# uncbiag/OAI_analysis_2

Measured on AMD Instinct MI355X. Metric: knee MRI volumes/sec (segment+register), 384x384x160 fp32, higher is better.
Workload: dtype fp16x3 (every fp32 value held as 2 fp16 terms = 22 mantissa bits, 3 MFMA passes per product, fp32 accumulate; fp32 in and out of every entry point; full-size parity vs the reference in `parity`)

## Files before the change

oai_analysis_2_amd/csrc/icon.hip:

```cpp
#include <cmath>
#include <cstring>
#include <vector>

#include "common.h"

namespace {

constexpr int kDown[6] = {2, 16, 32, 64, 256, 512};
constexpr int kUpOut[5] = {16, 32, 64, 128, 256};
constexpr int kUpIn[5] = {48, 96, 192, 512, 512};
constexpr float kLeaky = 0.01f;
constexpr float kBnEps = 1e-5f;
constexpr long long kSplitKBelow = 16384;
constexpr long long kMfmaUpFrom = 2048;
#ifndef OAI_LAST_XT
#define OAI_LAST_XT 2
#endif
constexpr long long kFewBlocks = 1024;

__device__ __forceinline__ float leaky(float v) { return v > 0.0f ? v : v * kLeaky; }

struct __attribute__((packed, aligned(4))) pair_f32s { float a, b; };
__device__ __forceinline__ void pair_store(float* p, float a, float b) { *reinterpret_cast<pair_f32s*>(p) = pair_f32s{a, b}; }

// ... 66 lines not shown

__device__ __forceinline__ void up_src(int dst, int in_size, int& i0, int& i1, float& l0, float& l1) {
    float src = 0.5f * ((float)dst + 0.5f) - 0.5f;
    src = src < 0.0f ? 0.0f : src;
    i0 = (int)src;
    i1 = i0 + (i0 < in_size - 1 ? 1 : 0);
    l1 = src - (float)i0;
    l0 = 1.0f - l1;
}

template <int COUT_T, int KS>
__global__ void __launch_bounds__(256)
icon_up_kernel(const float* __restrict__ x, int Cin, int D, int H, int W,
               const float* __restrict__ wk , const float* __restrict__ bias,
               const float* __restrict__ bn_scale, const float* __restrict__ bn_shift,
               float* __restrict__ out, int Cout, int Dc, int Hc, int Wc) {
    constexpr int VT = 256 / KS;
    __shared__ float red[KS > 1 ? (KS - 1) * VT * COUT_T : 1];
    const int cg = blockIdx.y;
    const int ks = KS == 1 ? 0 : threadIdx.x / VT;
    const int par = blockIdx.z, pz = par >> 2, py = (par >> 1) & 1, px = par & 1;
    const int nz = (Dc - pz + 1) / 2, ny = (Hc - py + 1) / 2, nx = (Wc - px + 1) / 2;
    const long long nv = (long long)nz * ny * nx;
    const long long v = (long long)blockIdx.x * VT + threadIdx.x % VT;
    const bool live = v < nv;
    const long long vv = live ? v : 0;
    const int tx = (int)(vv % nx), ty = (int)((vv / nx) % ny), tz = (int)(vv / ((long long)nx * ny));
    const int oz = 2 * tz + pz, oy = 2 * ty + py, ox = 2 * tx + px;
    const long long plane = (long long)D * H * W;
    const long long oplane = (long long)Dc * Hc * Wc;
    const int qz = (pz + 1) & 1, qy = (py + 1) & 1, qx = (px + 1) & 1;
    float acc[COUT_T];
#pragma unroll
    for (int j = 0; j < COUT_T; ++j) acc[j] = 0.0f;
    if (KS == 1 && !live) return;
    if (KS == 1 || live)
        for (int ci = ks; ci < Cin; ci += KS) {
            const float* xp = x + ci * plane;
            const float* wp = wk + ((long long)ci * 64) * Cout + cg * COUT_T;
#pragma unroll 8
            for (int t = 0; t < 8; ++t) {
                const int kz = qz + 2 * (t >> 2), ky = qy + 2 * ((t >> 1) & 1), kx = qx + 2 * (t & 1);
                const int iz = (oz + 1 - kz) >> 1, iy = (oy + 1 - ky) >> 1, ix = (ox + 1 - kx) >> 1;
                float in = 0.0f;
                if ((unsigned)iz < (unsigned)D && (unsigned)iy < (unsigned)H && (unsigned)ix < (unsigned)W)
                    in = leaky(xp[((long long)iz * H + iy) * W + ix]);
                const float* w = wp + ((kz * 4 + ky) * 4 + kx) * Cout;
#pragma unroll
                for (int j = 0; j < COUT_T; ++j) acc[j] = fmaf(in, w[j], acc[j]);
            }
        }
    if (KS > 1) {
        if (ks > 0) {
#pragma unroll
            for (int j = 0; j < COUT_T; ++j) red[((ks - 1) * COUT_T + j) * VT + threadIdx.x % VT] = acc[j];
        }
        __syncthreads();
        if (ks > 0) return;
#pragma unroll
        for (int k = 1; k < KS; ++k)
#pragma unroll
            for (int j = 0; j < COUT_T; ++j) acc[j] += red[((k - 1) * COUT_T + j) * VT + threadIdx.x];
    }
    if (!live) return;
    int z0, z1, y0, y1, x0, x1;
    float a0, a1, b0, b1, c0, c1;
    up_src(oz, D, z0, z1, a0, a1);
    up_src(oy, H, y0, y1, b0, b1);
    up_src(ox, W, x0, x1, c0, c1);
#pragma unroll
    for (int j = 0; j < COUT_T; ++j) {
        const int co = cg * COUT_T + j;
        const float* p = x + co * plane;
        auto at = [&](int zz, int yy, int xx) { return p[((long long)zz * H + yy) * W + xx]; };
        const float res = a0 * (b0 * (c0 * at(z0, y0, x0) + c1 * at(z0, y0, x1)) + b1 * (c0 * at(z0, y1, x0) + c1 * at(z0, y1, x1))) +
                          a1 * (b0 * (c0 * at(z1, y0, x0) + c1 * at(z1, y0, x1)) + b1 * (c0 * at(z1, y1, x0) + c1 * at(z1, y1, x1)));
        const float r = (acc[j] + bias[co]) + res;
        out[co * oplane + ((long long)oz * Hc + oy) * Wc + ox] = r * bn_scale[co] + bn_shift[co];
    }
}

typedef float f32x4m __attribute__((ext_vector_type(4)));

template <int MB, bool SPLIT>
__global__ void __launch_bounds__(256)
icon_up_mfma_kernel(const float* __restrict__ x, int Cin, int D, int H, int W,
                    const float* __restrict__ wk , const float* __restrict__ bias,
                    const float* __restrict__ bn_scale, const float* __restrict__ bn_shift,
                    float* __restrict__ out, int Cout, int Dc, int Hc, int Wc, int ntxb, long long nunits) {
    __shared__ float red[SPLIT ? 3 * MB * 2 * 4 * 64 : 1];
    const int lane = threadIdx.x & 63, wave = threadIdx.x >> 6;
    const long long unit = SPLIT ? (long long)blockIdx.x : (long long)blockIdx.x * 4 + wave;
    if (unit >= nunits) return;
    const int txb = (int)(unit % ntxb);
    const int rowi = (int)(unit / ntxb);
    const int oy = rowi % Hc, oz = rowi / Hc;
    const int co0 = blockIdx.y * 16;
    const int pz = oz & 1, py = oy & 1, tz = oz >> 1, ty = oy >> 1;
    const int col = lane & 15, kq = lane >> 4;
    const long long plane = (long long)D * H * W;
    f32x4m acc[MB][2];
#pragma unroll
    for (int m = 0; m < MB; ++m)
#pragma unroll
        for (int p = 0; p < 2; ++p) acc[m][p] = f32x4m{0.0f, 0.0f, 0.0f, 0.0f};
    const int tx0 = txb * MB * 16 + col;
    for (int a = SPLIT ? (wave >> 1) : 0; a < (SPLIT ? (wave >> 1) + 1 : 2); ++a) {
        const int kz = pz ? 2 * a : 1 + 2 * a, iz = pz ? tz + 1 - a : tz - a;
        if ((unsigned)iz >= (unsigned)D) continue;
        for (int b = SPLIT ? (wave & 1) : 0; b < (SPLIT ? (wave & 1) + 1 : 2); ++b) {
            const int ky = py ? 2 * b : 1 + 2 * b, iy = py ? ty + 1 - b : ty - b;
            if ((unsigned)iy >= (unsigned)H) continue;
            const float* xrow = x + ((long long)iz * H + iy) * W;
            const float* wt = wk + (long long)((kz * 4 + ky) * 4) * Cout + co0 + col;
            for (int ci0 = 0; ci0 < Cin; ci0 += 4) {
                const int ci = ci0 + kq;
                const float* wp = wt + (long long)ci * 64 * Cout;
                const float w0 = wp[0], w1 = wp[Cout], w2 = wp[2 * Cout], w3 = wp[3 * Cout];
                const float* xp = xrow + ci * plane;
                float xm[MB], xc[MB], xq[MB];
#pragma unroll
                for (int m = 0; m < MB; ++m) {
                    const int tx = tx0 + m * 16;
                    xm[m] = (unsigned)(tx - 1) < (unsigned)W ? leaky(xp[tx - 1]) : 0.0f;
                    xc[m] = tx < W ? leaky(xp[tx]) : 0.0f;
                    xq[m] = tx + 1 < W ? leaky(xp[tx + 1]) : 0.0f;
                }
#pragma unroll
                for (int m = 0; m < MB; ++m) {
                    acc[m][0] = __builtin_amdgcn_mfma_f32_16x16x4f32(w1, xc[m], acc[m][0], 0, 0, 0);
                    acc[m][1] = __builtin_amdgcn_mfma_f32_16x16x4f32(w0, xq[m], acc[m][1], 0, 0, 0);
                }
#pragma unroll
                for (int m = 0; m < MB; ++m) {
                    acc[m][0] = __builtin_amdgcn_mfma_f32_16x16x4f32(w3, xm[m], acc[m][0], 0, 0, 0);
                    acc[m][1] = __builtin_amdgcn_mfma_f32_16x16x4f32(w2, xc[m], acc[m][1], 0, 0, 0);
                }
            }
        }
    }
    if constexpr (SPLIT) {
        if (wave > 0) {
#pragma unroll
            for (int m = 0; m < MB; ++m)
#pragma unroll
                for (int p = 0; p < 2; ++p)
#pragma unroll
                    for (int r = 0; r < 4; ++r) red[((((wave - 1) * MB + m) * 2 + p) * 4 + r) * 64 + lane] = acc[m][p][r];
        }
        __syncthreads();
        if (wave > 0) return;
#pragma unroll
        for (int w = 0; w < 3; ++w)
#pragma unroll
            for (int m = 0; m < MB; ++m)
#pragma unroll
                for (int p = 0; p < 2; ++p)
#pragma unroll
                    for (int r = 0; r < 4; ++r) acc[m][p][r] += red[(((w * MB + m) * 2 + p) * 4 + r) * 64 + lane];
    }
    int z0, z1, y0, y1;
    float a0, a1, b0, b1;
    up_src(oz, D, z0, z1, a0, a1);
    up_src(oy, H, y0, y1, b0, b1);
    const long long oplane = (long long)Dc * Hc * Wc;
    const int nxt = (Wc + 1) / 2;
#pragma unroll
    for (int m = 0; m < MB; ++m) {
        const int tx = tx0 + m * 16;
        if (tx >= nxt) continue;
#pragma unroll
        for (int r = 0; r < 4; ++r) {
            const int co = co0 + 4 * kq + r;
            const float* p = x + co * plane;
            auto at = [&](int zz, int yy, int xx) { return p[((long long)zz * H + yy) * W + xx]; };
            float v[2];
#pragma unroll
            for (int px = 0; px < 2; ++px) {
                int x0, x1;
                float c0, c1;
                up_src(2 * tx + px, W, x0, x1, c0, c1);
                const float res = a0 * (b0 * (c0 * at(z0, y0, x0) + c1 * at(z0, y0, x1)) + b1 * (c0 * at(z0, y1, x0) + c1 * at(z0, y1, x1))) +
                                  a1 * (b0 * (c0 * at(z1, y0, x0) + c1 * at(z1, y0, x1)) + b1 * (c0 * at(z1, y1, x0) + c1 * at(z1, y1, x1)));
                const float t = (acc[m][px][r] + bias[co]) + res;
                v[px] = t * bn_scale[co] + bn_shift[co];
            }
            float* o = out + co * oplane + ((long long)oz * Hc + oy) * Wc + 2 * tx;
            if (2 * tx + 1 < Wc) { pair_store(o, v[0], v[1]); }
            else o[0] = v[0];
        }
    }
}

template <int XT>
__global__ void __launch_bounds__(256)
icon_last_conv_kernel(const float* __restrict__ x, int Cin, int D, int H, int W,
                      const float* __restrict__ wk , const float* __restrict__ bias, float* __restrict__ out, float div) {
    const int nxq = (W + XT - 1) / XT;
    const long long total = (long long)D * H * nxq;
    const long long id = (long long)blockIdx.x * 256 + threadIdx.x;
    if (id >= total) return;
    const int xq = (int)(id % nxq);
    const int y = (int)((id / nxq) % H), z = (int)(id / ((long long)nxq * H));
    const int xs = XT * xq;
    const long long plane = (long long)D * H * W;
    float acc[XT][3];
#pragma unroll
    for (int v = 0; v < XT; ++v)
#pragma unroll
        for (int j = 0; j < 3; ++j) acc[v][j] = 0.0f;
    for (int ci = 0; ci < Cin; ++ci) {
        const float* xp = x + ci * plane;
        const float* wp = wk + (long long)ci * 27 * 3;
#pragma unroll
        for (int dz = 0; dz < 3; ++dz)
#pragma unroll
            for (int dy = 0; dy < 3; ++dy) {
                const int iz = z + dz - 1, iy = y + dy - 1;
                const bool rowok = (unsigned)iz < (unsigned)D && (unsigned)iy < (unsigned)H;
                const float* rp = xp + ((long long)(rowok ? iz : 0) * H + (rowok ? iy : 0)) * W;
                float in[XT + 2];
#pragma unroll
                for (int e = 0; e < XT + 2; ++e) {
                    const int ix = xs - 1 + e;
                    in[e] = rowok && (unsigned)ix < (unsigned)W ? rp[ix] : 0.0f;
                }
#pragma unroll
                for (int dx = 0; dx < 3; ++dx) {
                    const float* w = wp + ((dz * 3 + dy) * 3 + dx) * 3;
#pragma unroll
                    for (int v = 0; v < XT; ++v)
#pragma unroll
                        for (int j = 0; j < 3; ++j) acc[v][j] = fmaf(in[v + dx], w[j], acc[v][j]);
                }
            }
    }
#pragma unroll
    for (int j = 0; j < 3; ++j)
#pragma unroll
        for (int v = 0; v < XT; ++v)
            if (xs + v < W) {
                const float r = acc[v][j] + bias[j];
                out[j * plane + ((long long)z * H + y) * W + xs + v] = div == 1.0f ? r : r / div;
            }
}

__global__ void __launch_bounds__(256) copy_f32_kernel(const float* __restrict__ src, float* __restrict__ dst, long long n) {
    const long long n4 = n >> 2;
    const long long stride = (long long)gridDim.x * 256;
    if (((reinterpret_cast<size_t>(src) | reinterpret_cast<size_t>(dst)) & 15) == 0) {
        for (long long i = (long long)blockIdx.x * 256 + threadIdx.x; i < n4; i += stride)
            reinterpret_cast<float4*>(dst)[i] = reinterpret_cast<const float4*>(src)[i];
        for (long long i = 4 * n4 + (long long)blockIdx.x * 256 + threadIdx.x; i < n; i += stride) dst[i] = src[i];
    } else {
        for (long long i = (long long)blockIdx.x * 256 + threadIdx.x; i < n; i += stride) dst[i] = src[i];
    }
}

int copy_f32(const float* src, float* dst, long long n, hipStream_t st) {
    long long blocks = (n / 4 + 255) / 256;
    if (blocks < 1) blocks = 1;
    if (blocks > 4096) blocks = 4096;
    copy_f32_kernel<<<(unsigned)blocks, 256, 0, st>>>(src, dst, n);
    OAI_CHECK_LAUNCH();
    return OAI_OK;
}

struct NetWeights {
    float* down_w[5]; float* down_b[5];
    float* up_w[5]; float* up_b[5]; float* bn_s[5]; float* bn_t[5];
    float* last_w; float* last_b;
};

}

struct IconStep {
    enum Kind { POOL, UNET, CHAIN } kind;
    int lvl = 0;
    int net = -1;
    size_t src = 0, src2 = 0, dst = 0;
    bool has_start = false, has_image = false;
    size_t start = 0;
    int nf = 0;
    size_t field[OAI_WARP_CHAIN_MAX_FIELDS];
    int field_lvl[OAI_WARP_CHAIN_MAX_FIELDS];
};

struct oai_icon {
    std::vector<NetWeights> net;
    std::vector<oai_icon_node> nodes;
    int root = 0;
    int D, H, W;
    std::vector<void*> allocs;
    std::vector<IconStep> steps;
    size_t off_A = 0, off_B = 0, off_phi = 0, off_unet = 0, ws_floats = 0;
    int nets_at_level[8] = {0, 0, 0, 0, 0, 0, 0, 0};
    int chain_len = 0;
    bool use_graph = true, graph_broken = false;
    bool pad_front = true;
    hipStream_t cap_stream = nullptr;
    hipGraphExec_t gexec = nullptr;
    void* g_ws = nullptr;
    long long replays = 0, direct_runs = 0;
};

namespace {

int upload(oai_icon* h, const std::vector<float>& v, float** dst) {
    void* d = nullptr;
    OAI_CHECK_HIP(hipMalloc(&d, v.size() * sizeof(float)));
    h->allocs.push_back(d);
    OAI_CHECK_HIP(hipMemcpy(d, v.data(), v.size() * sizeof(float), hipMemcpyHostToDevice));
    *dst = (float*)d;
    return OAI_OK;
}

std::vector<float> repack_conv(const float* w, int co_n, int ci_n, int taps) {
    std::vector<float> o((size_t)co_n * ci_n * taps);
    for (int co = 0; co < co_n; ++co)
        for (int ci = 0; ci < ci_n; ++ci)
            for (int t = 0; t < taps; ++t) o[((size_t)ci * taps + t) * co_n + co] = w[((size_t)co * ci_n + ci) * taps + t];
    return o;
}
std::vector<float> repack_convT(const float* w, int ci_n, int co_n, int taps) {
    std::vector<float> o((size_t)co_n * ci_n * taps);
    for (int ci = 0; ci < ci_n; ++ci)
        for (int co = 0; co < co_n; ++co)
            for (int t = 0; t < taps; ++t) o[((size_t)ci * taps + t) * co_n + co] = w[((size_t)ci * co_n + co) * taps + t];
    return o;
}

struct Dims { int d[6][3]; long long vox[6]; };

Dims level_dims(int D, int H, int W) {
    Dims r;
    r.d[0][0] = D; r.d[0][1] = H; r.d[0][2] = W;
    for (int l = 1; l < 6; ++l) for (int i = 0; i < 3; ++i) r.d[l][i] = (r.d[l - 1][i] + 1) / 2;
    for (int l = 0; l < 6; ++l) r.vox[l] = (long long)r.d[l][0] * r.d[l][1] * r.d[l][2];
    return r;
}

size_t unet_carve(float* ws, const Dims& dm, float* cat[5], float*& bottom) {
    oai::Ws w(ws);
    for (int l = 0; l < 5; ++l) cat[l] = w.take<float>((size_t)(kUpOut[l] + kDown[l]) * dm.vox[l]);
    bottom = w.take<float>((size_t)kDown[5] * dm.vox[5]);
    return w.off / 4;
}

size_t unet_ws_floats(int D, int H, int W) {
    float *cat[5], *bottom;
    return unet_carve(nullptr, level_dims(D, H, W), cat, bottom);
}

int unet_forward(const NetWeights& nw, bool pad_front, const float* a, const float* b, int D, int H, int W, float* out,
                 float* ws, hipStream_t st) {
    const Dims dm = level_dims(D, H, W);
    float *cat[5], *bottom;
    unet_carve(ws, dm, cat, bottom);
    if (int rc = copy_f32(a, cat[0] + (size_t)kUpOut[0] * dm.vox[0], dm.vox[0], st)) return rc;
    if (int rc = copy_f32(b, cat[0] + (size_t)(kUpOut[0] + 1) * dm.vox[0], dm.vox[0], st)) return rc;
    for (int l = 0; l < 5; ++l) {
        const float* src = cat[l] + (size_t)kUpOut[l] * dm.vox[l];
        float* dst = l < 4 ? cat[l + 1] + (size_t)kUpOut[l + 1] * dm.vox[l + 1] : bottom;
        const int res_ofs = pad_front ? kDown[l + 1] - kDown[l] : 0;
        auto launch = [&](auto kernel, dim3 grid) {
            kernel<<<grid, 256, 0, st>>>(src, kDown[l], dm.d[l][0], dm.d[l][1], dm.d[l][2], nw.down_w[l], nw.down_b[l], dst, kDown[l + 1],
                                         dm.d[l + 1][0], dm.d[l + 1][1], dm.d[l + 1][2], 1.0f, res_ofs);
        };
        if (dm.vox[l + 1] >= kSplitKBelow || kDown[l] < 8) {
            launch(icon_conv3_kernel<2, 16, true, true, 1>, dim3(oai::cdiv(dm.vox[l + 1], 256), kDown[l + 1] / 16));
        } else if ((long long)oai::cdiv(dm.vox[l + 1], 32) * (kDown[l + 1] / 16) >= kFewBlocks) {
            launch(icon_conv3_kernel<2, 16, true, true, 8>, dim3(oai::cdiv(dm.vox[l + 1], 32), kDown[l + 1] / 16));
        } else if ((long long)oai::cdiv(dm.vox[l + 1], 32) * (kDown[l + 1] / 16) < kFewBlocks / 16) {
            launch(icon_conv3_kernel<2, 1, true, true, 8>, dim3(oai::cdiv(dm.vox[l + 1], 32), kDown[l + 1]));
        } else {
            launch(icon_conv3_kernel<2, 4, true, true, 8>, dim3(oai::cdiv(dm.vox[l + 1], 32), kDown[l + 1] / 4));
        }
        OAI_CHECK_LAUNCH();
    }
    for (int l = 4; l >= 0; --l) {
        const float* src = l == 4 ? bottom : cat[l + 1];
        const long long per_par = (long long)((dm.d[l][0] + 1) / 2) * ((dm.d[l][1] + 1) / 2) * ((dm.d[l][2] + 1) / 2);
        auto launch = [&](auto kernel, dim3 grid, auto... tail) {
            kernel<<<grid, 256, 0, st>>>(src, kUpIn[l], dm.d[l + 1][0], dm.d[l + 1][1], dm.d[l + 1][2], nw.up_w[l], nw.up_b[l], nw.bn_s[l], nw.bn_t[l],
                                         cat[l], kUpOut[l], dm.d[l][0], dm.d[l][1], dm.d[l][2], tail...);
        };
        if (per_par >= kMfmaUpFrom) {
            constexpr int MB = 2;
            const int ntxb = (int)oai::cdiv((dm.d[l][2] + 1) / 2, 16 * MB);
            const long long nunits = (long long)dm.d[l][0] * dm.d[l][1] * ntxb;
            launch(icon_up_mfma_kernel<MB, false>, dim3(oai::cdiv(nunits, 4), kUpOut[l] / 16), ntxb, nunits);
        } else if (kUpOut[l] % 16 == 0 && kUpIn[l] % 4 == 0) {
            constexpr int MB = 1;
            const int ntxb = (int)oai::cdiv((dm.d[l][2] + 1) / 2, 16 * MB);
            const long long nunits = (long long)dm.d[l][0] * dm.d[l][1] * ntxb;
            launch(icon_up_mfma_kernel<MB, true>, dim3((unsigned)nunits, kUpOut[l] / 16), ntxb, nunits);
        } else if ((long long)oai::cdiv(per_par, 32) * (kUpOut[l] / 16) * 8 >= kFewBlocks) {
            launch(icon_up_kernel<16, 8>, dim3(oai::cdiv(per_par, 32), kUpOut[l] / 16, 8));
        } else if ((long long)oai::cdiv(per_par, 32) * (kUpOut[l] / 16) * 8 < kFewBlocks / 16) {
            launch(icon_up_kernel<1, 8>, dim3(oai::cdiv(per_par, 32), kUpOut[l], 8));
        } else {
            launch(icon_up_kernel<4, 8>, dim3(oai::cdiv(per_par, 32), kUpOut[l] / 4, 8));
        }
        OAI_CHECK_LAUNCH();
    }
    constexpr int XT = OAI_LAST_XT;
    icon_last_conv_kernel<XT><<<oai::cdiv((long long)D * H * ((W + XT - 1) / XT), 256), 256, 0, st>>>(cat[0], kUpOut[0] + kDown[0], D, H, W,
                                                                                                     nw.last_w, nw.last_b, out, 10.0f);
    OAI_CHECK_LAUNCH();
    return OAI_OK;
}

bool dims_ok(int D, int H, int W) {
    const Dims dm = level_dims(D, H, W);
    for (int i = 0; i < 3; ++i)
        if (dm.d[4][i] < 2) return false;
    return true;
}

struct Link { size_t off; int lvl; };

struct TreePlanner {
    oai_icon* h;
    long long vox[8];
    int gd[8][3];
    oai::Ws ws{nullptr};
    std::vector<std::pair<std::pair<size_t, int>, size_t>> pooled;
    std::vector<char> node_used, net_used;
    int err = OAI_OK;

    size_t take(size_t floats) { const size_t o = ws.off / 4; ws.take<float>(floats); return o; }

    int fail(const char* msg, int v) { if (!err) err = oai::set_error(OAI_ERR_ARG, msg, v); return err; }

    size_t pool(size_t src, int lvl) {
        for (auto& e : pooled) if (e.first.first == src && e.first.second == lvl) return e.second;
        IconStep st; st.kind = IconStep::POOL; st.lvl = lvl; st.src = src; st.dst = take(vox[lvl + 1]);
        h->steps.push_back(st);
        pooled.push_back({{src, lvl}, st.dst});
        return st.dst;
    }

    void chain(const std::vector<Link>& F, int lvl, bool has_image, size_t image, size_t out) {
        IconStep st; st.kind = IconStep::CHAIN; st.lvl = lvl; st.dst = out; st.has_image = has_image; st.src = image;
        size_t i = 0;
        if (!F.empty() && F[0].lvl == lvl) { st.has_start = true; st.start = F[0].off; i = 1; }
        for (; i < F.size(); ++i) { st.field[st.nf] = F[i].off; st.field_lvl[st.nf] = F[i].lvl; ++st.nf; }
        h->steps.push_back(st);
    }

    std::vector<Link> eval(int node, size_t A, size_t B, int lvl, int depth) {
        std::vector<Link> none;
        if (err) return none;
        if (node < 0 || node >= (int)h->nodes.size()) { fail("oai_icon_create: node index %d out of range", node); return none; }
        if (depth > 32 || node_used[node]) { fail("oai_icon_create: node %d is used twice (the step tree must be a tree)", node); return none; }
        node_used[node] = 1;
        const oai_icon_node nd = h->nodes[node];
        if (nd.kind == OAI_ICON_FFVF) {
            if (nd.a < 0 || nd.a >= (int)h->net.size()) { fail("oai_icon_create: FFVF names net %d, which does not exist", nd.a); return none; }
            if (net_used[nd.a]) { fail("oai_icon_create: net %d is used by two FFVF nodes", nd.a); return none; }
            net_used[nd.a] = 1;
            if (!dims_ok(gd[lvl][0], gd[lvl][1], gd[lvl][2])) {
                fail("oai_icon_create: the grid of net %d is too small for five 2x poolings (each axis must be >= 17)", nd.a);
                return none;
            }
            IconStep st; st.kind = IconStep::UNET; st.lvl = lvl; st.net = nd.a; st.src = A; st.src2 = B; st.dst = take(3 * vox[lvl]);
            h->steps.push_back(st);
            ++h->nets_at_level[lvl];
            return {Link{st.dst, lvl}};
        }
// ... 1 lines not shown
            if (lvl + 1 >= 8 || gd[lvl][0] < 2 || gd[lvl][1] < 2 || gd[lvl][2] < 2) { fail("oai_icon_create: too many Downsample levels at node %d", node); return none; }
            const size_t a = pool(A, lvl), b = pool(B, lvl);
            return eval(nd.a, a, b, lvl + 1, depth + 1);
        }
        if (nd.kind == OAI_ICON_TWO) {
            std::vector<Link> Fphi = eval(nd.a, A, B, lvl, depth + 1);
            if (err) return none;
            const size_t Aw = take(vox[lvl]);
            if ((int)Fphi.size() > OAI_WARP_CHAIN_MAX_FIELDS) { fail("oai_icon_create: more than %d steps in one chain", OAI_WARP_CHAIN_MAX_FIELDS); return none; }
            chain(Fphi, lvl, true, A, Aw);
            std::vector<Link> F = eval(nd.b, Aw, B, lvl, depth + 1);
            if (err) return none;
            F.insert(F.end(), Fphi.begin(), Fphi.end());
            return F;
        }
        fail("oai_icon_create: node %d has an unknown kind", node);
        return none;
    }
};

int plan_tree(oai_icon* h) {
    TreePlanner P;
    P.h = h;
    int d = h->D, hh = h->H, w = h->W;
    for (int l = 0; l < 8; ++l) {
        P.gd[l][0] = d; P.gd[l][1] = hh; P.gd[l][2] = w;
        P.vox[l] = (long long)d * hh * w;
        d = (d + 1) / 2; hh = (hh + 1) / 2; w = (w + 1) / 2;
    }
    P.node_used.assign(h->nodes.size(), 0);
    P.net_used.assign(h->net.size(), 0);
    h->steps.clear();
    h->off_A = P.take(P.vox[0]); h->off_B = P.take(P.vox[0]);
    std::vector<Link> F = P.eval(h->root, h->off_A, h->off_B, 0, 0);
    if (P.err) return P.err;
    if ((int)F.size() > OAI_WARP_CHAIN_MAX_FIELDS)
        return oai::set_error(OAI_ERR_ARG, "oai_icon_create: %d steps in the final chain (limit %d)", (int)F.size(), OAI_WARP_CHAIN_MAX_FIELDS);
    for (size_t n = 0; n < P.net_used.size(); ++n)
        if (!P.net_used[n]) return oai::set_error(OAI_ERR_ARG, "oai_icon_create: net %d is not used by the step tree", (int)n);
    for (size_t n = 0; n < P.node_used.size(); ++n)
        if (!P.node_used[n]) return oai::set_error(OAI_ERR_ARG, "oai_icon_create: node %d is not reachable from the root", (int)n);
    h->off_phi = P.take(3 * P.vox[0]);
    P.chain(F, 0, false, 0, h->off_phi);
    h->chain_len = (int)F.size();
    int top = 0;
    while (top < 8 && !h->nets_at_level[top]) ++top;
    h->off_unet = P.take(unet_ws_floats(P.gd[top][0], P.gd[top][1], P.gd[top][2]));
    h->ws_floats = P.ws.off / 4;
    return OAI_OK;
}

}

extern "C" {

int oai_icon_create(const oai_icon_unet_params* nets, int n_nets, const oai_icon_node* nodes, int n_nodes, int root,
                    int D, int H, int W, oai_icon** out) {
    OAI_CHECK_ARG(nets && nodes && out, "oai_icon_create: null pointer");
    OAI_CHECK_ARG(n_nets >= 1 && n_nets <= OAI_WARP_CHAIN_MAX_FIELDS, "oai_icon_create: 1..%d U-Nets", OAI_WARP_CHAIN_MAX_FIELDS);
    OAI_CHECK_ARG(n_nodes >= 1 && n_nodes <= 64 && root >= 0 && root < n_nodes, "oai_icon_create: bad node list");
    OAI_CHECK_ARG(D > 1 && H > 1 && W > 1, "oai_icon_create: bad network shape");
    oai_icon* h = new oai_icon();
    h->D = D; h->H = H; h->W = W;
    h->net.resize(n_nets);
    h->nodes.assign(nodes, nodes + n_nodes);
    h->root = root;
    int rc = plan_tree(h);
    for (int n = 0; n < n_nets && rc == OAI_OK; ++n) {
        const oai_icon_unet_params& p = nets[n];
        NetWeights& nw = h->net[n];
        for (int l = 0; l < 5 && rc == OAI_OK; ++l) {
            if (!p.down_w[l] || !p.down_b[l] || !p.up_w[l] || !p.up_b[l]) {
                rc = oai::set_error(OAI_ERR_ARG, "oai_icon_create: net %d level %d has a null parameter", n, l);
                break;
            }
            const int nbn = (p.bn_gamma[l] != nullptr) + (p.bn_beta[l] != nullptr) + (p.bn_mean[l] != nullptr) + (p.bn_var[l] != nullptr);
            if (nbn != 0 && nbn != 4) {
                rc = oai::set_error(OAI_ERR_ARG, "oai_icon_create: net %d level %d: BatchNorm needs gamma, beta, mean and var (or none of them)", n, l);
                break;
            }
            if ((rc = upload(h, repack_conv(p.down_w[l], kDown[l + 1], kDown[l], 27), &nw.down_w[l]))) break;
            if ((rc = upload(h, std::vector<float>(p.down_b[l], p.down_b[l] + kDown[l + 1]), &nw.down_b[l]))) break;
            if ((rc = upload(h, repack_convT(p.up_w[l], kUpIn[l], kUpOut[l], 64), &nw.up_w[l]))) break;
            if ((rc = upload(h, std::vector<float>(p.up_b[l], p.up_b[l] + kUpOut[l]), &nw.up_b[l]))) break;
            std::vector<float> s(kUpOut[l]), t(kUpOut[l]);
            for (int c = 0; c < kUpOut[l]; ++c) {
                s[c] = nbn ? p.bn_gamma[l][c] / sqrtf(p.bn_var[l][c] + kBnEps) : 1.0f;
                t[c] = nbn ? p.bn_beta[l][c] - p.bn_mean[l][c] * s[c] : 0.0f;
            }
            if ((rc = upload(h, s, &nw.bn_s[l]))) break;
            if ((rc = upload(h, t, &nw.bn_t[l]))) break;
        }
        if (rc) break;
        if (!p.last_w || !p.last_b) { rc = oai::set_error(OAI_ERR_ARG, "oai_icon_create: net %d lastConv is null", n); break; }
        if ((rc = upload(h, repack_conv(p.last_w, 3, 18, 27), &nw.last_w))) break;
        if ((rc = upload(h, std::vector<float>(p.last_b, p.last_b + 3), &nw.last_b))) break;
    }
    if (rc) { oai_icon_destroy(h); return rc; }
    *out = h;
    return OAI_OK;
}

void oai_icon_destroy(oai_icon* h) {
    if (!h) return;
    if (h->gexec) (void)hipGraphExecDestroy(h->gexec);
    if (h->cap_stream) (void)hipStreamDestroy(h->cap_stream);
    for (void* p : h->allocs) (void)hipFree(p);
    delete h;
}

size_t oai_icon_workspace_bytes(const oai_icon* h) {
    if (!h) return 0;
    return h->ws_floats * sizeof(float);
}

int oai_icon_describe(const oai_icon* h, int* n_nets, int* levels, int* chain_len) {
    OAI_CHECK_ARG(h, "oai_icon_describe: null handle");
    if (n_nets) *n_nets = (int)h->net.size();
    if (levels) for (int l = 0; l < 8; ++l) levels[l] = h->nets_at_level[l];
    if (chain_len) *chain_len = h->chain_len;
    return OAI_OK;
}

int oai_icon_unet_forward(oai_icon* h, int which, const float* a, const float* b, int D, int H, int W, float* out,
                          void* ws, size_t ws_bytes, void* stream) {
    OAI_CHECK_ARG(h && a && b && out && ws, "oai_icon_unet_forward: null pointer");
    OAI_CHECK_ARG(which >= 0 && which < (int)h->net.size(), "oai_icon_unet_forward: net index must be 0..%d", (int)h->net.size() - 1);
    OAI_CHECK_ARG(dims_ok(D, H, W), "oai_icon_unet_forward: %dx%dx%d too small for five 2x poolings (each axis >= 17)", D, H, W);
    OAI_CHECK_WORKSPACE("oai_icon_unet_forward", ws_bytes, unet_ws_floats(D, H, W) * 4);
    return unet_forward(h->net[which], h->pad_front, a, b, D, H, W, out, (float*)ws, (hipStream_t)stream);
}

static int icon_forward_body(oai_icon* h, float* ws, hipStream_t st) {
    int gd[8][3];
    int d = h->D, hh = h->H, w = h->W;
    for (int l = 0; l < 8; ++l) { gd[l][0] = d; gd[l][1] = hh; gd[l][2] = w; d = (d + 1) / 2; hh = (hh + 1) / 2; w = (w + 1) / 2; }
    for (const IconStep& s : h->steps) {
        const int* g = gd[s.lvl];
        int rc = OAI_OK;
        if (s.kind == IconStep::POOL) {
            rc = oai_avgpool2_3d(ws + s.src, 1, g[0], g[1], g[2], ws + s.dst, st);
        } else if (s.kind == IconStep::UNET) {
            rc = unet_forward(h->net[s.net], h->pad_front, ws + s.src, ws + s.src2, g[0], g[1], g[2], ws + s.dst, ws + h->off_unet, st);
        } else {
            const float* f[OAI_WARP_CHAIN_MAX_FIELDS];
            int fdims[3 * OAI_WARP_CHAIN_MAX_FIELDS];
            for (int i = 0; i < s.nf; ++i) {
                f[i] = ws + s.field[i];
                for (int k = 0; k < 3; ++k) fdims[3 * i + k] = gd[s.field_lvl[i]][k];
            }
            rc = oai_warp_chain(s.has_start ? ws + s.start : nullptr, g[0], g[1], g[2], s.nf, f, fdims,
                                s.has_image ? ws + s.src : nullptr, g[0], g[1], g[2], ws + s.dst, st);
        }
        if (rc) return rc;
    }
    return OAI_OK;
}

int oai_icon_forward(oai_icon* h, const float* A, const float* B, float* phi, void* ws, size_t ws_bytes, void* stream) {
    OAI_CHECK_ARG(h && A && B && phi && ws, "oai_icon_forward: null pointer");
    const long long vh = (long long)h->D * h->H * h->W;
    OAI_CHECK_WORKSPACE("oai_icon_forward", ws_bytes, h->ws_floats * sizeof(float));
    hipStream_t st = (hipStream_t)stream;
    float* wsf = (float*)ws;
    if (int rc = copy_f32(A, wsf + h->off_A, vh, st)) return rc;
    if (int rc = copy_f32(B, wsf + h->off_B, vh, st)) return rc;
    bool replayed = false;
    if (h->use_graph && !h->graph_broken) {
        if (!h->gexec || h->g_ws != ws) {
            if (h->gexec) { (void)hipGraphExecDestroy(h->gexec); h->gexec = nullptr; }
            if (!h->cap_stream && hipStreamCreateWithFlags(&h->cap_stream, hipStreamNonBlocking) != hipSuccess) h->graph_broken = true;
            hipGraph_t g = nullptr;
            if (!h->graph_broken && hipStreamBeginCapture(h->cap_stream, hipStreamCaptureModeThreadLocal) == hipSuccess) {
                const int rc = icon_forward_body(h, wsf, h->cap_stream);
                const hipError_t e = hipStreamEndCapture(h->cap_stream, &g);
                if (rc != OAI_OK || e != hipSuccess || !g || hipGraphInstantiate(&h->gexec, g, nullptr, nullptr, 0) != hipSuccess) {
                    h->gexec = nullptr;
                    h->graph_broken = true;
                }
                if (g) (void)hipGraphDestroy(g);
                (void)hipGetLastError();
            } else h->graph_broken = true;
            h->g_ws = ws;
        }
        if (h->gexec) {
            OAI_CHECK_HIP(hipGraphLaunch(h->gexec, st));
            ++h->replays;
            replayed = true;
        }
    }
    if (!replayed) {
        if (int rc = icon_forward_body(h, wsf, st)) return rc;
        ++h->direct_runs;
    }
    return copy_f32(wsf + h->off_phi, phi, 3 * vh, st);
}

int oai_icon_set_graph(oai_icon* h, int enable) {
    OAI_CHECK_ARG(h, "oai_icon_set_graph: null handle");
    h->use_graph = enable != 0;
    return OAI_OK;
}

int oai_icon_set_option(oai_icon* h, const char* name, int value) {
    OAI_CHECK_ARG(h && name, "oai_icon_set_option: null pointer");
    if (!strcmp(name, "pad_front")) {
        OAI_CHECK_ARG(value == 0 || value == 1, "oai_icon_set_option: pad_front must be 0 or 1");
        if (h->pad_front != (value != 0)) {
            h->pad_front = value != 0;
            if (h->gexec) { (void)hipGraphExecDestroy(h->gexec); h->gexec = nullptr; }
            h->g_ws = nullptr;
        }
        return OAI_OK;
    }
    return oai::set_error(OAI_ERR_ARG, "oai_icon_set_option: unknown option '%s'", name);
}

int oai_icon_graph_info(const oai_icon* h, int* captured, long long* replays, long long* direct_runs) {
    OAI_CHECK_ARG(h, "oai_icon_graph_info: null handle");
    if (captured) *captured = h->gexec ? 1 : (h->graph_broken ? -1 : 0);
    if (replays) *replays = h->replays;
    if (direct_runs) *direct_runs = h->direct_runs;
    return OAI_OK;
}

}
```

oai_analysis_2_amd/registration.py:

```python
from __future__ import annotations

from dataclasses import dataclass
from typing import Dict, Optional, Sequence, Tuple

import numpy as np
import torch

from . import _lib, ops
from .image import Image, as_image

NET_SHAPE = (80, 192, 192)


def network_affine(img: Image, net_shape_dhw: Sequence[int]):
    size = img.size_xyz.astype(np.float64)
    shape = np.asarray(net_shape_dhw[::-1], np.float64)
    M = img.direction @ np.diag(img.spacing * (size / shape))
    c_net = (shape - 1.0) / 2.0
    c_img = img.origin + img.direction @ (img.spacing * (size - 1.0) / 2.0)
    return M, c_net, c_img


def resample_affines(image_A: Image, image_B: Image, net_shape_dhw: Sequence[int]):
    M_A, c_net, c_A = network_affine(image_A, net_shape_dhw)
# ... 121 lines not shown
        sd = {k[len("regis_net."):]: v for k, v in sd.items() if k.startswith("regis_net.")}
    params = {k: v for k, v in sd.items() if k.rsplit(".", 1)[-1] not in _BUFFER_LEAVES}
    tree = parse_icon_tree(params.keys())
    expected = set()
    for pre in tree.net_prefixes:
        for d in range(5):
            expected |= {f"{pre}downConvs.{d}.weight", f"{pre}downConvs.{d}.bias", f"{pre}upConvs.{d}.weight", f"{pre}upConvs.{d}.bias"}
            expected |= {f"{pre}batchNorms.{d}.{n}" for n in ("weight", "bias", "running_mean", "running_var")}
        expected |= {f"{pre}lastConv.weight", f"{pre}lastConv.bias"}
    unknown = sorted(set(params) - expected)
    if unknown:
        raise KeyError(f"unexpected keys in the ICON state_dict: {unknown[:4]}")
    missing = sorted(k for k in expected - set(params) if ".batchNorms." not in k)
    if missing:
        raise KeyError(f"ICON state_dict is missing {missing[:4]}")
    for pre in tree.net_prefixes:
        if tuple(params[f"{pre}downConvs.0.weight"].shape) != (16, 2, 3, 3, 3) or tuple(params[f"{pre}lastConv.weight"].shape) != (3, 18, 3, 3, 3) \
                or tuple(params[f"{pre}upConvs.4.weight"].shape) != (512, 256, 4, 4, 4):
            raise KeyError(f"'{pre}' is not a 3-D tallUNet2 (channel widths differ)")
    return (params, tree) if with_tree else params


class IconEngine:

    def __init__(self, state_dict: Dict[str, torch.Tensor], net_shape: Sequence[int] = NET_SHAPE, device=None,
                 apply_bn: Optional[bool] = None, pad_front: bool = True):
        import ctypes as C
        if apply_bn is None:
            apply_bn, self.apply_bn_reason = infer_apply_bn(state_dict)
        else:
            self.apply_bn_reason = "stated by the caller"
        state_dict, self.tree = map_icon_state_dict(state_dict, with_tree=True)
        self.lib = _lib.load()
        if not torch.cuda.is_available():
            raise _lib.OaiError("no HIP device: the MI355X path has no CPU fallback")
        self.device = torch.device(device) if device is not None else torch.device("cuda", torch.cuda.current_device())
        self.net_shape = tuple(int(v) for v in net_shape)
        keep = []

        def ptr(key):
            if key not in state_dict:
                raise KeyError(f"ICON state_dict is missing {key}")
            t = state_dict[key].detach().to("cpu", torch.float32).contiguous()
            keep.append(t)
            return t.data_ptr()

        n_nets = len(self.tree.net_prefixes)
        params = (_lib.IconUnetParams * n_nets)()
        for n, pre in enumerate(self.tree.net_prefixes):
            p = params[n]
            for d in range(5):
                p.down_w[d], p.down_b[d] = ptr(f"{pre}downConvs.{d}.weight"), ptr(f"{pre}downConvs.{d}.bias")
                p.up_w[d], p.up_b[d] = ptr(f"{pre}upConvs.{d}.weight"), ptr(f"{pre}upConvs.{d}.bias")
                if apply_bn:
                    p.bn_gamma[d], p.bn_beta[d] = ptr(f"{pre}batchNorms.{d}.weight"), ptr(f"{pre}batchNorms.{d}.bias")
                    p.bn_mean[d], p.bn_var[d] = ptr(f"{pre}batchNorms.{d}.running_mean"), ptr(f"{pre}batchNorms.{d}.running_var")
            p.last_w, p.last_b = ptr(f"{pre}lastConv.weight"), ptr(f"{pre}lastConv.bias")
        nodes = (_lib.IconNode * len(self.tree.nodes))(*[_lib.IconNode(*nd) for nd in self.tree.nodes])
        handle = C.c_void_p()
        _lib.call("oai_icon_create", params, n_nets, nodes, len(self.tree.nodes), self.tree.root, *self.net_shape, C.byref(handle),
                  device=self.device)
        self._h = handle
        self.n_nets = n_nets
        self.apply_bn, self.pad_front = bool(apply_bn), bool(pad_front)
        if not pad_front:
            _lib.call("oai_icon_set_option", self._h, b"pad_front", 0)
        self._ws = _lib.workspace("oai_icon", self.device, self._h)

    def __del__(self):
        h = getattr(self, "_h", None)
        if h:
            self.lib.oai_icon_destroy(h)
            self._h = None

    def describe(self):
        import ctypes as C
        n, lv, cl = C.c_int(), (C.c_int * 8)(), C.c_int()
        _lib.call("oai_icon_describe", self._h, C.byref(n), lv, C.byref(cl))
        return n.value, list(lv), cl.value

    def set_graph(self, enable: bool) -> None:
        _lib.call("oai_icon_set_graph", self._h, int(enable))

    def graph_info(self):
        import ctypes as C
        cap, rep, dr = C.c_int(), C.c_longlong(), C.c_longlong()
        _lib.call("oai_icon_graph_info", self._h, C.byref(cap), C.byref(rep), C.byref(dr))
        return cap.value, rep.value, dr.value

    def unet(self, which: int, a: torch.Tensor, b: torch.Tensor) -> torch.Tensor:
        a = a.to(self.device, torch.float32).contiguous()
        b = b.to(self.device, torch.float32).contiguous()
        D, H, W = a.shape
        out = torch.empty((3, D, H, W), dtype=torch.float32, device=self.device)
        _lib.call("oai_icon_unet_forward", self._h, which, a.data_ptr(), b.data_ptr(), D, H, W, out.data_ptr(), self._ws.data_ptr(),
                  self._ws.numel(), _lib.STREAM, device=self.device)
        return out

    def phi(self, A_net: torch.Tensor, B_net: torch.Tensor) -> torch.Tensor:
        A_net = A_net.to(self.device, torch.float32).contiguous()
        B_net = B_net.to(self.device, torch.float32).contiguous()
        if tuple(A_net.shape) != self.net_shape or tuple(B_net.shape) != self.net_shape:
            raise ValueError(f"images must be resized to the network shape {self.net_shape}")
        out = torch.empty((3, *self.net_shape), dtype=torch.float32, device=self.device)
        _lib.call("oai_icon_forward", self._h, A_net.data_ptr(), B_net.data_ptr(), out.data_ptr(), self._ws.data_ptr(), self._ws.numel(),
                  _lib.STREAM, device=self.device)
        return out

    def register_pair(self, image_A: torch.Tensor, image_B: torch.Tensor, both: bool = False):
        A = ops.resize_trilinear(image_A.to(self.device, torch.float32)[None], self.net_shape)[0]
        B = ops.resize_trilinear(image_B.to(self.device, torch.float32)[None], self.net_shape)[0]
        phi_AB = self.phi(A, B)
        phi_BA = self.phi(B, A) if both else None
        return phi_AB, phi_BA


def _unwrap_state_dict(state_dict):
    sd = state_dict
    for wrap in ("model_state_dict", "state_dict"):
        if wrap in sd and isinstance(sd[wrap], dict):
            sd = sd[wrap]
    return sd


def _has_nontrivial_batchnorm(state_dict) -> bool:
    for k, v in _unwrap_state_dict(state_dict).items():
        if ".batchNorms." not in k and not k.startswith("batchNorms."):
            continue
        t = torch.as_tensor(v).float()
        if k.endswith("num_batches_tracked"):
            continue
        want = 1.0 if (k.endswith(".weight") or k.endswith("running_var")) else 0.0
        if t.numel() and float((t - want).abs().max()) > 1e-6:
            return True
    return False


def infer_apply_bn(state_dict) -> Tuple[bool, str]:
    sd = _unwrap_state_dict(state_dict)
    tracked = [int(torch.as_tensor(v).max()) for k, v in sd.items()
               if k.endswith("num_batches_tracked") and (".batchNorms." in k or k.startswith("batchNorms.")) and torch.as_tensor(v).numel()]
    if any(n > 0 for n in tracked):
        return True, f"num_batches_tracked = {max(tracked)} > 0: the BatchNorm layers were called in training"
    if _has_nontrivial_batchnorm(sd):
        return True, "BatchNorm tensors differ from their constructor values: the layers were trained, hence called"
    return False, "BatchNorm tensors are pristine (never called in training): applying them would change phi by < 1e-4"


_BN_NOTED = False


def _note_bn_decision_once(apply_bn: bool, reason: str) -> None:
    global _BN_NOTED
    if _BN_NOTED:
        return
    _BN_NOTED = True
    print(f"ICON_Registration: apply_bn={apply_bn} decided from the checkpoint -- {reason}")


class ICON_Registration:

    def __init__(self, weights=None, net_shape: Sequence[int] = NET_SHAPE, device=None, verbose: bool = True,
                 apply_bn: Optional[bool] = None, pad_front: bool = True):
        import os
        if weights is None:
            root = os.environ.get("OAI_DATA_DIR")
# ... 45 lines not shown
```

Measured before the change: 7.884.

## Add LDS-staged MFMA transposed-conv kernel for the three finest ICON up levels

Adds a transposed-convolution kernel for the first three U-Net up levels. Each block handles one output parity and a group of output channels. Weights are repacked at load time into MFMA fragment order and double-buffered through LDS in chunks shared by all four waves. Input loads are software-pipelined, and DPP row rotates build the neighbouring-x operands instead of extra global loads. The aim is to cut redundant weight and input traffic and raise MFMA utilisation, at the cost of extra weight memory, LDS use and a more complex code path behind a new up_staged option.

Result: no change. 7.945, median of 6 (+0.8%).

```diff
diff --git a/oai_analysis_2_amd/csrc/icon.hip b/oai_analysis_2_amd/csrc/icon.hip
--- a/oai_analysis_2_amd/csrc/icon.hip
+++ b/oai_analysis_2_amd/csrc/icon.hip
@@ -172,6 +172,45 @@
 
 typedef float f32x4m __attribute__((ext_vector_type(4)));
 
+template <int MB>
+__device__ __forceinline__ void up_mfma_epilogue(const f32x4m (&acc)[MB][2], const float* __restrict__ x, int D, int H, int W,
+                                                 const float* __restrict__ bias, const float* __restrict__ bn_scale,
+                                                 const float* __restrict__ bn_shift, float* __restrict__ out, int Dc, int Hc, int Wc,
+                                                 int oz, int oy, int tx0, int co0, int kq) {
+    const long long plane = (long long)D * H * W;
+    int z0, z1, y0, y1;
+    float a0, a1, b0, b1;
+    up_src(oz, D, z0, z1, a0, a1);
+    up_src(oy, H, y0, y1, b0, b1);
+    const long long oplane = (long long)Dc * Hc * Wc;
+    const int nxt = (Wc + 1) / 2;
+#pragma unroll
+    for (int m = 0; m < MB; ++m) {
+        const int tx = tx0 + m * 16;
+        if (tx >= nxt) continue;
+#pragma unroll
+        for (int r = 0; r < 4; ++r) {
+            const int co = co0 + 4 * kq + r;
+            const float* p = x + co * plane;
+            auto at = [&](int zz, int yy, int xx) { return p[((long long)zz * H + yy) * W + xx]; };
+            float v[2];
+#pragma unroll
+            for (int px = 0; px < 2; ++px) {
+                int x0, x1;
+                float c0, c1;
+                up_src(2 * tx + px, W, x0, x1, c0, c1);
+                const float res = a0 * (b0 * (c0 * at(z0, y0, x0) + c1 * at(z0, y0, x1)) + b1 * (c0 * at(z0, y1, x0) + c1 * at(z0, y1, x1))) +
+                                  a1 * (b0 * (c0 * at(z1, y0, x0) + c1 * at(z1, y0, x1)) + b1 * (c0 * at(z1, y1, x0) + c1 * at(z1, y1, x1)));
+                const float t = (acc[m][px][r] + bias[co]) + res;
+                v[px] = t * bn_scale[co] + bn_shift[co];
+            }
+            float* o = out + co * oplane + ((long long)oz * Hc + oy) * Wc + 2 * tx;
+            if (2 * tx + 1 < Wc) { pair_store(o, v[0], v[1]); }
+            else o[0] = v[0];
+        }
+    }
+}
+
 template <int MB, bool SPLIT>
 __global__ void __launch_bounds__(256)
 icon_up_mfma_kernel(const float* __restrict__ x, int Cin, int D, int H, int W,
@@ -249,37 +288,142 @@
 #pragma unroll
                     for (int r = 0; r < 4; ++r) acc[m][p][r] += red[(((w * MB + m) * 2 + p) * 4 + r) * 64 + lane];
     }
-    int z0, z1, y0, y1;
-    float a0, a1, b0, b1;
-    up_src(oz, D, z0, z1, a0, a1);
-    up_src(oy, H, y0, y1, b0, b1);
-    const long long oplane = (long long)Dc * Hc * Wc;
-    const int nxt = (Wc + 1) / 2;
-#pragma unroll
-    for (int m = 0; m < MB; ++m) {
-        const int tx = tx0 + m * 16;
-        if (tx >= nxt) continue;
-#pragma unroll
-        for (int r = 0; r < 4; ++r) {
-            const int co = co0 + 4 * kq + r;
-            const float* p = x + co * plane;
-            auto at = [&](int zz, int yy, int xx) { return p[((long long)zz * H + yy) * W + xx]; };
-            float v[2];
-#pragma unroll
-            for (int px = 0; px < 2; ++px) {
-                int x0, x1;
-                float c0, c1;
-                up_src(2 * tx + px, W, x0, x1, c0, c1);
-                const float res = a0 * (b0 * (c0 * at(z0, y0, x0) + c1 * at(z0, y0, x1)) + b1 * (c0 * at(z0, y1, x0) + c1 * at(z0, y1, x1))) +
-                                  a1 * (b0 * (c0 * at(z1, y0, x0) + c1 * at(z1, y0, x1)) + b1 * (c0 * at(z1, y1, x0) + c1 * at(z1, y1, x1)));
-                const float t = (acc[m][px][r] + bias[co]) + res;
-                v[px] = t * bn_scale[co] + bn_shift[co];
-            }
-            float* o = out + co * oplane + ((long long)oz * Hc + oy) * Wc + 2 * tx;
-            if (2 * tx + 1 < Wc) { pair_store(o, v[0], v[1]); }
-            else o[0] = v[0];
-        }
-    }
+    up_mfma_epilogue<MB>(acc, x, D, H, W, bias, bn_scale, bn_shift, out, Dc, Hc, Wc, oz, oy, tx0, co0, kq);
+}
+
+constexpr int kUpStagedLevels = 3;
+constexpr int kUpChunkFloats = 3072;
+
+template <int CTRL>
+__device__ __forceinline__ float row_rotate(float v) {
+    return __builtin_bit_cast(float, __builtin_amdgcn_update_dpp(0, __builtin_bit_cast(int, v), CTRL, 0xf, 0xf, false));
+}
+
+template <int NCB>
+__global__ void __launch_bounds__(256)
+icon_up_staged_kernel(const float* __restrict__ x, int Cin, int D, int H, int W,
+                      const f32x4m* __restrict__ wf , const float* __restrict__ bias,
+                      const float* __restrict__ bn_scale, const float* __restrict__ bn_shift,
+                      float* __restrict__ out, int Cout, int Dc, int Hc, int Wc, int ntxb) {
+    constexpr int MB = 2, KC = 48 / NCB, STEPS = KC / 4;
+    constexpr int C4 = KC * NCB * 16;
+    static_assert(C4 * 4 == kUpChunkFloats && C4 == 3 * 256, "a chunk is three float4 per thread");
+    __shared__ f32x4m wlds[2][C4];
+    const int lane = threadIdx.x & 63, wave = threadIdx.x >> 6;
+    const int par = blockIdx.y & 3, cg = blockIdx.y >> 2, ncg = gridDim.y >> 2;
+    const int pz = par >> 1, py = par & 1;
+    const int nyp = (Hc - py + 1) / 2;
+    const long long nunits = (long long)((Dc - pz + 1) / 2) * nyp * ntxb;
+    if ((long long)blockIdx.x * 4 >= nunits) return;
+    const long long unit = (long long)blockIdx.x * 4 + wave;
+    const bool live = unit < nunits;
+    const long long u = live ? unit : 0;
+    const int txb = (int)(u % ntxb);
+    const int rowi = (int)(u / ntxb);
+    const int ty = rowi % nyp, tz = rowi / nyp;
+    const int oy = 2 * ty + py, oz = 2 * tz + pz;
+    const int col = lane & 15, kq = lane >> 4;
+    const long long plane = (long long)D * H * W;
+    f32x4m acc[NCB][MB][2];
+#pragma unroll
+    for (int cb = 0; cb < NCB; ++cb)
+#pragma unroll
+        for (int m = 0; m < MB; ++m)
+#pragma unroll
+            for (int p = 0; p < 2; ++p) acc[cb][m][p] = f32x4m{0.0f, 0.0f, 0.0f, 0.0f};
+    const int tx0 = txb * MB * 16 + col;
+    const int hx = col == 0 ? tx0 - 1 : tx0 + 17;
+    const bool halo = (col == 0 || col == 15) && (unsigned)hx < (unsigned)W;
+    const int i0 = min(tx0, W - 1), i1 = min(tx0 + 16, W - 1), ih = halo ? hx : i0;
+    const bool in0 = tx0 < W, in1 = tx0 + 16 < W;
+    unsigned hmask = halo ? ~0u : 0u;
+    asm volatile("" : "+v"(hmask));
+    const int nck = Cin / KC;
+    auto chunk_src = [&](int t, int k) {
+        const int a = t >> 1, b = t & 1;
+        const int kz = pz ? 2 * a : 1 + 2 * a, ky = py ? 2 * b : 1 + 2 * b;
+        return wf + ((long long)((kz * 4 + ky) * ncg + cg) * (Cin / 4)) * (NCB * 64) + (long long)k * C4 + threadIdx.x;
+    };
+    auto row_ok = [&](int t) {
+        const int iz = pz ? tz + 1 - (t >> 1) : tz - (t >> 1), iy = py ? ty + 1 - (t & 1) : ty - (t & 1);
+        return live && (unsigned)iz < (unsigned)D && (unsigned)iy < (unsigned)H;
+    };
+    auto row_ptr = [&](int t) {
+        const int iz = pz ? tz + 1 - (t >> 1) : tz - (t >> 1), iy = py ? ty + 1 - (t & 1) : ty - (t & 1);
+        return x + ((long long)min(max(iz, 0), D - 1) * H + min(max(iy, 0), H - 1)) * W + kq * plane;
+    };
+    constexpr int G = 3, GPC = STEPS / G;
+    static_assert(STEPS % G == 0, "a chunk is a whole number of groups");
+    auto load_group = [&](float (&v)[G][3], int t, int k, int gi) {
+        const float* xr = row_ptr(t) + (long long)(k * KC + gi * 4 * G) * plane;
+#pragma unroll
+        for (int j = 0; j < G; ++j) {
+            const float* xp = xr + 4 * j * plane;
+            v[j][0] = xp[i0];
+            v[j][1] = xp[i1];
+            v[j][2] = xp[ih];
+        }
+    };
+    {
+        const f32x4m* s = chunk_src(0, 0);
+        const f32x4m s0 = s[0], s1 = s[256], s2 = s[512];
+        f32x4m* d = wlds[0] + threadIdx.x;
+        d[0] = s0; d[256] = s1; d[512] = s2;
+    }
+    float cur[G][3], nxt[G][3];
+    load_group(cur, 0, 0, 0);
+    for (int t = 0, c = 0; t < 4; ++t) {
+        const bool ok = row_ok(t);
+        for (int k = 0; k < nck; ++k, ++c) {
+            __syncthreads();
+            const bool last_k = k + 1 == nck, last = last_k && t == 3;
+            const int tn = last ? t : last_k ? t + 1 : t, kn = last ? k : last_k ? 0 : k + 1;
+            const f32x4m* sn = chunk_src(tn, kn);
+            const f32x4m s0 = sn[0], s1 = sn[256], s2 = sn[512];
+            const f32x4m* wl = wlds[c & 1] + lane;
+#pragma unroll
+            for (int gi = 0; gi < GPC; ++gi) {
+                if (gi + 1 < GPC) load_group(nxt, t, k, gi + 1);
+                else load_group(nxt, tn, kn, 0);
+                if (ok) {
+#pragma unroll
+                    for (int j = 0; j < G; ++j) {
+                        const int s = gi * G + j;
+                        const float c0 = in0 ? leaky(cur[j][0]) : 0.0f, c1 = in1 ? leaky(cur[j][1]) : 0.0f, hv = __builtin_bit_cast(float, __builtin_bit_cast(unsigned, leaky(cur[j][2])) & hmask);
+                        const float r0 = row_rotate<0x121>(c0), r1 = row_rotate<0x121>(c1);
+                        const float l0 = row_rotate<0x12f>(c0), l1 = row_rotate<0x12f>(c1);
+                        const float xc[MB] = {c0, c1};
+                        const float xm[MB] = {col == 0 ? hv : r0, col == 0 ? r0 : r1};
+                        const float xq[MB] = {col == 15 ? l1 : l0, col == 15 ? hv : l1};
+#pragma unroll
+                        for (int cb = 0; cb < NCB; ++cb) {
+                            const f32x4m w = wl[(s * NCB + cb) * 64];
+#pragma unroll
+                            for (int m = 0; m < MB; ++m) {
+                                acc[cb][m][0] = __builtin_amdgcn_mfma_f32_16x16x4f32(w.y, xc[m], acc[cb][m][0], 0, 0, 0);
+                                acc[cb][m][1] = __builtin_amdgcn_mfma_f32_16x16x4f32(w.x, xq[m], acc[cb][m][1], 0, 0, 0);
+                            }
+#pragma unroll
+                            for (int m = 0; m < MB; ++m) {
+                                acc[cb][m][0] = __builtin_amdgcn_mfma_f32_16x16x4f32(w.w, xm[m], acc[cb][m][0], 0, 0, 0);
+                                acc[cb][m][1] = __builtin_amdgcn_mfma_f32_16x16x4f32(w.z, xc[m], acc[cb][m][1], 0, 0, 0);
+                            }
+                        }
+                    }
+                }
+#pragma unroll
+                for (int j = 0; j < G; ++j)
+#pragma unroll
+                    for (int e = 0; e < 3; ++e) cur[j][e] = nxt[j][e];
+            }
+            f32x4m* d = wlds[(c + 1) & 1] + threadIdx.x;
+            d[0] = s0; d[256] = s1; d[512] = s2;
+        }
+    }
+    if (!live) return;
+#pragma unroll
+    for (int cb = 0; cb < NCB; ++cb)
+        up_mfma_epilogue<MB>(acc[cb], x, D, H, W, bias, bn_scale, bn_shift, out, Dc, Hc, Wc, oz, oy, tx0, (cg * NCB + cb) * 16, kq);
 }
 
 template <int XT>
@@ -359,6 +503,7 @@
 struct NetWeights {
     float* down_w[5]; float* down_b[5];
     float* up_w[5]; float* up_b[5]; float* bn_s[5]; float* bn_t[5];
+    float* up_wf[kUpStagedLevels];
     float* last_w; float* last_b;
 };
 
@@ -388,6 +533,7 @@
     int chain_len = 0;
     bool use_graph = true, graph_broken = false;
     bool pad_front = true;
+    bool up_staged = true;
     hipStream_t cap_stream = nullptr;
     hipGraphExec_t gexec = nullptr;
     void* g_ws = nullptr;
@@ -420,6 +566,25 @@
     return o;
 }
 
+constexpr int up_ncb(int cout) { return cout >= 64 ? 4 : cout / 16; }
+static_assert(kUpIn[0] % (48 / up_ncb(kUpOut[0])) == 0 && kUpIn[1] % (48 / up_ncb(kUpOut[1])) == 0 && kUpIn[2] % (48 / up_ncb(kUpOut[2])) == 0,
+              "a tap pair's channels are a whole number of staged chunks");
+std::vector<float> repack_convT_frag(const float* w, int ci_n, int co_n) {
+    const int ncb = up_ncb(co_n), ncg = co_n / (16 * ncb);
+    std::vector<float> o((size_t)co_n * ci_n * 64);
+    size_t i = 0;
+    for (int tp = 0; tp < 16; ++tp)
+        for (int cg = 0; cg < ncg; ++cg)
+            for (int s = 0; s < ci_n / 4; ++s)
+                for (int cb = 0; cb < ncb; ++cb)
+                    for (int lane = 0; lane < 64; ++lane)
+                        for (int kx = 0; kx < 4; ++kx) {
+                            const int ci = 4 * s + (lane >> 4), co = (cg * ncb + cb) * 16 + (lane & 15);
+                            o[i++] = w[((size_t)ci * co_n + co) * 64 + tp * 4 + kx];
+                        }
+    return o;
+}
+
 struct Dims { int d[6][3]; long long vox[6]; };
 
 Dims level_dims(int D, int H, int W) {
@@ -442,7 +607,7 @@
     return unet_carve(nullptr, level_dims(D, H, W), cat, bottom);
 }
 
-int unet_forward(const NetWeights& nw, bool pad_front, const float* a, const float* b, int D, int H, int W, float* out,
+int unet_forward(const NetWeights& nw, bool pad_front, bool up_staged, const float* a, const float* b, int D, int H, int W, float* out,
                  float* ws, hipStream_t st) {
     const Dims dm = level_dims(D, H, W);
     float *cat[5], *bottom;
@@ -475,7 +640,17 @@
             kernel<<<grid, 256, 0, st>>>(src, kUpIn[l], dm.d[l + 1][0], dm.d[l + 1][1], dm.d[l + 1][2], nw.up_w[l], nw.up_b[l], nw.bn_s[l], nw.bn_t[l],
                                          cat[l], kUpOut[l], dm.d[l][0], dm.d[l][1], dm.d[l][2], tail...);
         };
-        if (per_par >= kMfmaUpFrom) {
+        if (per_par >= kMfmaUpFrom && up_staged && l < kUpStagedLevels) {
+            const int ntxb = (int)oai::cdiv((dm.d[l][2] + 1) / 2, 32);
+            const dim3 grid(oai::cdiv(per_par / ((dm.d[l][2] + 1) / 2) * ntxb, 4), 4 * (kUpOut[l] / (16 * up_ncb(kUpOut[l]))));
+            auto staged = [&](auto kernel) {
+                kernel<<<grid, 256, 0, st>>>(src, kUpIn[l], dm.d[l + 1][0], dm.d[l + 1][1], dm.d[l + 1][2], (const f32x4m*)nw.up_wf[l], nw.up_b[l], nw.bn_s[l],
+                                             nw.bn_t[l], cat[l], kUpOut[l], dm.d[l][0], dm.d[l][1], dm.d[l][2], ntxb);
+            };
+            if (l == 0) staged(icon_up_staged_kernel<up_ncb(kUpOut[0])>);
+            else if (l == 1) staged(icon_up_staged_kernel<up_ncb(kUpOut[1])>);
+            else staged(icon_up_staged_kernel<up_ncb(kUpOut[2])>);
+        } else if (per_par >= kMfmaUpFrom) {
             constexpr int MB = 2;
             const int ntxb = (int)oai::cdiv((dm.d[l][2] + 1) / 2, 16 * MB);
             const long long nunits = (long long)dm.d[l][0] * dm.d[l][1] * ntxb;
@@ -643,6 +818,7 @@
             if ((rc = upload(h, repack_conv(p.down_w[l], kDown[l + 1], kDown[l], 27), &nw.down_w[l]))) break;
             if ((rc = upload(h, std::vector<float>(p.down_b[l], p.down_b[l] + kDown[l + 1]), &nw.down_b[l]))) break;
             if ((rc = upload(h, repack_convT(p.up_w[l], kUpIn[l], kUpOut[l], 64), &nw.up_w[l]))) break;
+            if (l < kUpStagedLevels && (rc = upload(h, repack_convT_frag(p.up_w[l], kUpIn[l], kUpOut[l]), &nw.up_wf[l]))) break;
             if ((rc = upload(h, std::vector<float>(p.up_b[l], p.up_b[l] + kUpOut[l]), &nw.up_b[l]))) break;
             std::vector<float> s(kUpOut[l]), t(kUpOut[l]);
             for (int c = 0; c < kUpOut[l]; ++c) {
@@ -689,7 +865,7 @@
     OAI_CHECK_ARG(which >= 0 && which < (int)h->net.size(), "oai_icon_unet_forward: net index must be 0..%d", (int)h->net.size() - 1);
     OAI_CHECK_ARG(dims_ok(D, H, W), "oai_icon_unet_forward: %dx%dx%d too small for five 2x poolings (each axis >= 17)", D, H, W);
     OAI_CHECK_WORKSPACE("oai_icon_unet_forward", ws_bytes, unet_ws_floats(D, H, W) * 4);
-    return unet_forward(h->net[which], h->pad_front, a, b, D, H, W, out, (float*)ws, (hipStream_t)stream);
+    return unet_forward(h->net[which], h->pad_front, h->up_staged, a, b, D, H, W, out, (float*)ws, (hipStream_t)stream);
 }
 
 static int icon_forward_body(oai_icon* h, float* ws, hipStream_t st) {
@@ -702,7 +878,7 @@
         if (s.kind == IconStep::POOL) {
             rc = oai_avgpool2_3d(ws + s.src, 1, g[0], g[1], g[2], ws + s.dst, st);
         } else if (s.kind == IconStep::UNET) {
-            rc = unet_forward(h->net[s.net], h->pad_front, ws + s.src, ws + s.src2, g[0], g[1], g[2], ws + s.dst, ws + h->off_unet, st);
+            rc = unet_forward(h->net[s.net], h->pad_front, h->up_staged, ws + s.src, ws + s.src2, g[0], g[1], g[2], ws + s.dst, ws + h->off_unet, st);
         } else {
             const float* f[OAI_WARP_CHAIN_MAX_FIELDS];
             int fdims[3 * OAI_WARP_CHAIN_MAX_FIELDS];
@@ -765,10 +941,11 @@
 
 int oai_icon_set_option(oai_icon* h, const char* name, int value) {
     OAI_CHECK_ARG(h && name, "oai_icon_set_option: null pointer");
-    if (!strcmp(name, "pad_front")) {
-        OAI_CHECK_ARG(value == 0 || value == 1, "oai_icon_set_option: pad_front must be 0 or 1");
-        if (h->pad_front != (value != 0)) {
-            h->pad_front = value != 0;
+    bool* opt = !strcmp(name, "pad_front") ? &h->pad_front : !strcmp(name, "up_staged") ? &h->up_staged : nullptr;
+    if (opt) {
+        OAI_CHECK_ARG(value == 0 || value == 1, "oai_icon_set_option: %s must be 0 or 1", name);
+        if (*opt != (value != 0)) {
+            *opt = value != 0;
             if (h->gexec) { (void)hipGraphExecDestroy(h->gexec); h->gexec = nullptr; }
             h->g_ws = nullptr;
         }
diff --git a/oai_analysis_2_amd/registration.py b/oai_analysis_2_amd/registration.py
--- a/oai_analysis_2_amd/registration.py
+++ b/oai_analysis_2_amd/registration.py
@@ -227,6 +227,11 @@
     def set_graph(self, enable: bool) -> None:
         _lib.call("oai_icon_set_graph", self._h, int(enable))
 
+    def set_option(self, name: str, value: int) -> None:
+        _lib.call("oai_icon_set_option", self._h, name.encode(), int(value))
+        if name == "pad_front":
+            self.pad_front = bool(value)
+
     def graph_info(self):
         import ctypes as C
         cap, rep, dr = C.c_int(), C.c_longlong(), C.c_longlong()
```
